# sandialabs/tenzing

Hardware: AMD Instinct MI355X
Metric: best-schedule iter time (ms) + MCTS search wall-clock, 3D halo-exchange 8 ranks (lower is better)
Workload: dtype fp64

## Files before the change

tenzing_amd/csrc/bind/module.cpp:

```cpp
#include <pybind11/functional.h>
#include <pybind11/numpy.h>
#include <pybind11/pybind11.h>
#include <pybind11/stl.h>

#include "core/benchmark.hpp"
#include "core/health.hpp"
#include "core/solve.hpp"
#include "hip/comm_ops.hpp"
#include "hip/hip_runtime.hpp"
#include "hip/rccl_comm.hpp"
#include "hip/rocsparse_spmv.hpp"
#include "kernels/kernels.hpp"
#include "workloads/workloads.hpp"

#include <hip/hip_runtime_api.h>

#include <csignal>
#include <cstdlib>
#include <execinfo.h>
#include <sstream>
#include <unistd.h>
#include <vector>

namespace py = pybind11;
// ... 1127 lines not shown
     "symmetric, strictly diagonally dominant band matrix (mirrored random_band_matrix off-diagonals, "
     "a_ii = 1 + sum |a_ij|) as (rowPtr, colInd, val)");
  py::class_<CgArgs>(m, "CgArgs")
      .def(py::init<>())
      .def_readwrite("m", &CgArgs::m)
      .def_readwrite("bw", &CgArgs::bw)
      .def_readwrite("nnz", &CgArgs::nnz)
      .def_readonly("nnz_actual", &CgArgs::nnz_actual)
      .def_readwrite("seed", &CgArgs::seed)
      .def_readwrite("matrix", &CgArgs::matrix)
      .def_readwrite("device", &CgArgs::device)
      .def_readwrite("form", &CgArgs::form)
      .def_readwrite("lanes", &CgArgs::lanes)
      .def_readwrite("rhs", &CgArgs::rhs)
      .def_readwrite("nrhs", &CgArgs::nrhs)
      .def_readwrite("rhs_first", &CgArgs::rhs_first)
      .def_readwrite("prefix", &CgArgs::prefix)
      .def_readwrite("rank", &CgArgs::rank)
      .def_readwrite("size", &CgArgs::size)
      .def("json", [](const CgArgs &a) { return a.json().dump(); });
  {
    auto f32 = [](const std::vector<float> &v) { return py::array_t<float>(py::ssize_t(v.size()), v.data()); };
    py::class_<ConjugateGradient, std::shared_ptr<ConjugateGradient>>(m, "ConjugateGradient")
        .def(py::init([](const CgArgs &a) { return std::make_shared<ConjugateGradient>(a); }), py::arg("args"))
        .def_property_readonly("args", &ConjugateGradient::args)
        .def("rows", &ConjugateGradient::rows)
        .def("matrix", [](const ConjugateGradient &c) {
          const CsrHost &a = c.matrix();
          return py::make_tuple(a.rowPtr, a.colInd, a.val);
        }, "the system matrix as (rowPtr, colInd, val)")
        .def("setup", &ConjugateGradient::setup, py::call_guard<py::gil_scoped_release>())
        .def("ready", &ConjugateGradient::ready)
        .def("add_to_graph", &ConjugateGradient::add_to_graph)
        .def("reset", &ConjugateGradient::reset, py::call_guard<py::gil_scoped_release>(),
             "x = 0, r = p = b, rr = b . b (synchronous)")
        .def("x", [f32](const ConjugateGradient &c, int col) { return f32(c.x(col)); }, py::arg("col") = 0,
             "column col (0 .. nrhs - 1) of x, de-interleaved; likewise r, p, b, rr, check and residual")
        .def("r", [f32](const ConjugateGradient &c, int col) { return f32(c.r(col)); }, py::arg("col") = 0)
        .def("p", [f32](const ConjugateGradient &c, int col) { return f32(c.p(col)); }, py::arg("col") = 0)
        .def("b", [f32](const ConjugateGradient &c, int col) { return f32(c.b(col)); }, py::arg("col") = 0)
        .def("rr", &ConjugateGradient::rr, py::arg("col") = 0,
             "r . r of the current residual (f64, the kernels' summation order)")
        .def("check", &ConjugateGradient::check, py::arg("k"), py::arg("col") = 0,
             py::call_guard<py::gil_scoped_release>(),
             "max |x - x_ref| / max |x_ref| against k host iterations in f64")
        .def("residual", &ConjugateGradient::residual, py::arg("col") = 0,
             py::call_guard<py::gil_scoped_release>(),
             "the true residual ||b - A x|| / ||b|| of the current x, in f64 on the host");
  }
  m.def("read_matrix_market", [](const std::string &path) {
    CsrHost a = read_matrix_market(path);
    return py::make_tuple(a.rows, a.cols, a.rowPtr, a.colInd, a.val);
  }, py::arg("path"));
  m.def("write_matrix_market", [](int64_t rows, int64_t cols, std::vector<int32_t> rowPtr,
                                  std::vector<int32_t> colInd, std::vector<float> val,
                                  const std::string &path) {
    CsrHost a;
    a.rows = rows;
    a.cols = cols;
    a.rowPtr = std::move(rowPtr);
    a.colInd = std::move(colInd);
    a.val = std::move(val);
    TZ_CHECK(int64_t(a.rowPtr.size()) == rows + 1 && a.colInd.size() == a.val.size() &&
                 int64_t(a.colInd.size()) == int64_t(a.rowPtr.back()),
             "inconsistent CSR arrays");
    write_matrix_market(a, path);
  }, py::arg("rows"), py::arg("cols"), py::arg("row_ptr"), py::arg("col_ind"), py::arg("val"), py::arg("path"));
  m.def("row_partition", &row_partition);

  auto k = m.def_submodule("kernels", "hand-written gfx950 kernels (raw device pointers)");
  k.def("box_copy", [](uintptr_t grid, py::dict d, bool unpack, uintptr_t s) {
    kern::box_copy(reinterpret_cast<double *>(grid), box_from_dict(d), unpack, P(s));
  }, py::arg("grid"), py::arg("box"), py::arg("unpack"), py::arg("stream") = 0);
  k.def("box_copy_many", [](uintptr_t grid, std::vector<py::dict> ds, bool unpack, uintptr_t s) {
    std::vector<kern::BoxDesc> bs;
    for (auto &d : ds) bs.push_back(box_from_dict(d));
    kern::box_copy_many(reinterpret_cast<double *>(grid), bs.data(), int(bs.size()), unpack, P(s));
  }, py::arg("grid"), py::arg("boxes"), py::arg("unpack"), py::arg("stream") = 0);
  k.def("csr_spmv", [](int n, uintptr_t rp, uintptr_t ci, uintptr_t v, uintptr_t x, uintptr_t y, int lanes, bool acc, uintptr_t s) {
    kern::csr_spmv(n, reinterpret_cast<const int32_t *>(rp), reinterpret_cast<const int32_t *>(ci),
                   reinterpret_cast<const float *>(v), reinterpret_cast<const float *>(x),
                   reinterpret_cast<float *>(y), lanes, acc, P(s));
  }, py::arg("n_rows"), py::arg("row_ptr"), py::arg("col_ind"), py::arg("val"), py::arg("x"), py::arg("y"),
     py::arg("lanes") = 0, py::arg("accumulate") = false, py::arg("stream") = 0);
  py::class_<RocsparseCsr, std::shared_ptr<RocsparseCsr>>(
      k, "RocsparseCsr", "rocSPARSE CSR SpMV (library comparison variant): y = A x on raw pointers")
      .def(py::init([](int64_t m, int64_t n, int64_t nnz, uintptr_t rp, uintptr_t ci, uintptr_t v,
                       uintptr_t x, uintptr_t y, const std::string &alg) {
             return std::make_shared<RocsparseCsr>(
                 m, n, nnz, reinterpret_cast<const int32_t *>(rp), reinterpret_cast<const int32_t *>(ci),
                 reinterpret_cast<const float *>(v), reinterpret_cast<const float *>(x),
                 reinterpret_cast<float *>(y), alg.c_str());
           }),
           py::arg("m"), py::arg("n"), py::arg("nnz"), py::arg("row_ptr"), py::arg("col_ind"),
           py::arg("val"), py::arg("x"), py::arg("y"), py::arg("alg") = "adaptive")
      .def("run", [](const RocsparseCsr &r, uintptr_t s, bool acc) { r.run(P(s), acc); },
           py::arg("stream") = 0, py::arg("accumulate") = false);
  k.def("stencil7", [](uintptr_t in, uintptr_t out, int64_t base, int row, int ny, int nz,
                       int nouter, int64_t sy, int64_t sz, int64_t so, int xs, double c0, double c1,
                       bool lds, uintptr_t s, int m0, int m1) {
    kern::StencilBox b;
    b.in = reinterpret_cast<const double *>(in);
    b.out = reinterpret_cast<double *>(out);
    b.base = base;
    b.row = row;
    b.ny = ny;
    b.nz = nz;
    b.nouter = nouter;
    b.sy = sy;
    b.sz = sz;
    b.so = so;
    b.xs = xs;
    b.c0 = c0;
    b.c1 = c1;
    b.m0 = m0;
    b.m1 = m1;
    kern::stencil7(b, lds, P(s));
  }, py::arg("in_"), py::arg("out"), py::arg("base"), py::arg("row"), py::arg("ny"), py::arg("nz"),
     py::arg("nouter"), py::arg("sy"), py::arg("sz"), py::arg("so"), py::arg("xs"),
     py::arg("c0") = 0.4, py::arg("c1") = 0.1, py::arg("lds") = true, py::arg("stream") = 0,
     py::arg("m0") = 0, py::arg("m1") = 0);
  k.def("stencil_thin", [](int row, int ny, int nz) {
    kern::StencilBox b;
    b.row = row;
    b.ny = ny;
    b.nz = nz;
    return kern::stencil_thin(b);
  }, py::arg("row"), py::arg("ny"), py::arg("nz"),
     "whether stencil7 sends a box of these extents to the one-thread-per-element kernel");
  k.def("stencil7_thin_many", [](uintptr_t in, uintptr_t out, std::vector<py::dict> ds, uintptr_t s) {
    std::vector<kern::StencilBox> bs;
    for (auto &d : ds) {
      kern::StencilBox b;
      b.in = reinterpret_cast<const double *>(in);
      b.out = reinterpret_cast<double *>(out);
      b.base = d["base"].cast<int64_t>();
      b.sy = d["sy"].cast<int64_t>();
      b.sz = d["sz"].cast<int64_t>();
      b.so = d["so"].cast<int64_t>();
      b.row = d["row"].cast<int>();
      b.ny = d["ny"].cast<int>();
      b.nz = d["nz"].cast<int>();
      b.nouter = d["nouter"].cast<int>();
      b.xs = d["xs"].cast<int>();
      if (d.contains("m0")) b.m0 = d["m0"].cast<int>();
      if (d.contains("m1")) b.m1 = d["m1"].cast<int>();
      if (d.contains("c0")) b.c0 = d["c0"].cast<double>();
      if (d.contains("c1")) b.c1 = d["c1"].cast<double>();
      bs.push_back(b);
    }
    kern::stencil7_thin_many(bs.data(), int(bs.size()), P(s));
  }, py::arg("in_"), py::arg("out"), py::arg("boxes"), py::arg("stream") = 0,
     "the one-thread-per-element kernel over a list of boxes (dicts of the StencilBox fields)");
  k.def("set_stencil_tuning", [](int ty, int zc, int pf, bool db) {
    TZ_CHECK(ty == 8 || ty == 16, "stencil ty must be 8 or 16");
    TZ_CHECK(zc == 16 || zc == 32 || zc == 64 || zc == 128, "stencil zc must be 16, 32, 64 or 128");
    TZ_CHECK(zc != 128 || pf == 1, "stencil zc 128 takes pf 1");
    TZ_CHECK(pf == 1 || pf == 2, "stencil pf must be 1 or 2");
    kern::stencil_tuning().ty = ty;
    kern::stencil_tuning().zc = zc;
    kern::stencil_tuning().pf = pf;
    kern::stencil_tuning().db = db;
  }, py::arg("ty") = 16, py::arg("zc") = 64, py::arg("pf") = 1, py::arg("db") = true);
  k.def("set_stencil_xcd_tiles", [](bool on) { kern::stencil_tuning().xcd_tiles = on; }, py::arg("on"),
        "stencil tiles in XCD-contiguous order (each XCD a contiguous range of tiles)");
  k.def("get_stencil_xcd_tiles", []() { return kern::stencil_tuning().xcd_tiles; });
  k.attr("CG_MAX_PARTIALS") = kern::kCgMaxPartials;
  k.attr("SPMV_ILP") = kern::kSpmvIlp;
  k.def("dot_partial_count", &kern::dot_partial_count, py::arg("n"));
  k.def("spmv_dot_partial_count", &kern::spmv_dot_partial_count, py::arg("n_rows"), py::arg("lanes"));
  k.def("dot_partials_f32", [](int64_t n, uintptr_t u, uintptr_t v, uintptr_t part, uintptr_t s) {
    kern::dot_partials_f32(n, reinterpret_cast<const float *>(u), reinterpret_cast<const float *>(v),
                           reinterpret_cast<double *>(part), P(s));
  }, py::arg("n"), py::arg("u"), py::arg("v"), py::arg("partials"), py::arg("stream") = 0);
  k.def("sum_partials_f64", [](uintptr_t part, int np, uintptr_t out, uintptr_t s) {
    kern::sum_partials_f64(reinterpret_cast<const double *>(part), np, reinterpret_cast<double *>(out), P(s));
  }, py::arg("partials"), py::arg("np"), py::arg("out"), py::arg("stream") = 0);
  k.def("cg_alpha", [](uintptr_t part, int np, uintptr_t rr, uintptr_t alpha, uintptr_t s) {
    kern::cg_alpha(reinterpret_cast<const double *>(part), np, reinterpret_cast<const double *>(rr),
                   reinterpret_cast<double *>(alpha), P(s));
  }, py::arg("partials_pq"), py::arg("np"), py::arg("rr"), py::arg("alpha"), py::arg("stream") = 0);
  k.def("cg_beta", [](uintptr_t part, int np, uintptr_t rr, uintptr_t beta, uintptr_t s) {
    kern::cg_beta(reinterpret_cast<const double *>(part), np, reinterpret_cast<double *>(rr),
                  reinterpret_cast<double *>(beta), P(s));
  }, py::arg("partials_rr"), py::arg("np"), py::arg("rr"), py::arg("beta"), py::arg("stream") = 0);
  k.def("axpy_dev_f32", [](int64_t n, uintptr_t sc, int sign, uintptr_t x, uintptr_t y, uintptr_t s) {
    kern::axpy_dev_f32(n, reinterpret_cast<const double *>(sc), sign, reinterpret_cast<const float *>(x),
                       reinterpret_cast<float *>(y), P(s));
  }, py::arg("n"), py::arg("scalar"), py::arg("sign"), py::arg("x"), py::arg("y"), py::arg("stream") = 0);
  k.def("xpay_dev_f32", [](int64_t n, uintptr_t sc, uintptr_t x, uintptr_t y, uintptr_t s) {
    kern::xpay_dev_f32(n, reinterpret_cast<const double *>(sc), reinterpret_cast<const float *>(x),
                       reinterpret_cast<float *>(y), P(s));
  }, py::arg("n"), py::arg("scalar"), py::arg("x"), py::arg("y"), py::arg("stream") = 0);
  k.def("csr_spmv_dot", [](int n, uintptr_t rp, uintptr_t ci, uintptr_t v, uintptr_t p, uintptr_t q, int lanes,
                           uintptr_t pq, uintptr_t prr, int npRr, uintptr_t rr, uintptr_t s) {
    kern::csr_spmv_dot(n, reinterpret_cast<const int32_t *>(rp), reinterpret_cast<const int32_t *>(ci),
                       reinterpret_cast<const float *>(v), reinterpret_cast<const float *>(p),
                       reinterpret_cast<float *>(q), lanes, reinterpret_cast<double *>(pq),
                       reinterpret_cast<const double *>(prr), npRr, reinterpret_cast<double *>(rr), P(s));
  }, py::arg("n_rows"), py::arg("row_ptr"), py::arg("col_ind"), py::arg("val"), py::arg("p"), py::arg("q"),
     py::arg("lanes"), py::arg("partials_pq"), py::arg("partials_rr") = 0, py::arg("np_rr") = 0,
     py::arg("rr") = 0, py::arg("stream") = 0);
  k.def("cg_fused_x", [](int64_t n, uintptr_t pq, int np, uintptr_t rr, uintptr_t p, uintptr_t x, uintptr_t s) {
    kern::cg_fused_x(n, reinterpret_cast<const double *>(pq), np, reinterpret_cast<const double *>(rr),
                     reinterpret_cast<const float *>(p), reinterpret_cast<float *>(x), P(s));
  }, py::arg("n"), py::arg("partials_pq"), py::arg("np"), py::arg("rr"), py::arg("p"), py::arg("x"),
     py::arg("stream") = 0);
  k.def("cg_fused_r", [](int64_t n, uintptr_t pq, int np, uintptr_t rr, uintptr_t q, uintptr_t r, uintptr_t prr,
                         uintptr_t s) {
    kern::cg_fused_r(n, reinterpret_cast<const double *>(pq), np, reinterpret_cast<const double *>(rr),
                     reinterpret_cast<const float *>(q), reinterpret_cast<float *>(r),
                     reinterpret_cast<double *>(prr), P(s));
  }, py::arg("n"), py::arg("partials_pq"), py::arg("np"), py::arg("rr"), py::arg("q"), py::arg("r"),
     py::arg("partials_rr"), py::arg("stream") = 0);
  k.def("cg_fused_p", [](int64_t n, uintptr_t prr, int np, uintptr_t rr, uintptr_t r, uintptr_t p, uintptr_t s) {
    kern::cg_fused_p(n, reinterpret_cast<const double *>(prr), np, reinterpret_cast<const double *>(rr),
                     reinterpret_cast<const float *>(r), reinterpret_cast<float *>(p), P(s));
  }, py::arg("n"), py::arg("partials_rr"), py::arg("np"), py::arg("rr"), py::arg("r"), py::arg("p"),
     py::arg("stream") = 0);
  k.def("csr_spmv_dot2", [](int n, uintptr_t rp, uintptr_t ci, uintptr_t v, uintptr_t r, uintptr_t w, int lanes,
                            uintptr_t pg, uintptr_t pd, uintptr_t gOut, uintptr_t aOut, uintptr_t gPrev,
                            uintptr_t aPrev, uintptr_t s) {
    kern::csr_spmv_dot2(n, reinterpret_cast<const int32_t *>(rp), reinterpret_cast<const int32_t *>(ci),
                        reinterpret_cast<const float *>(v), reinterpret_cast<const float *>(r),
                        reinterpret_cast<float *>(w), lanes, reinterpret_cast<double *>(pg),
                        reinterpret_cast<double *>(pd), reinterpret_cast<const double *>(gOut),
                        reinterpret_cast<const double *>(aOut), reinterpret_cast<double *>(gPrev),
                        reinterpret_cast<double *>(aPrev), P(s));
  }, py::arg("n_rows"), py::arg("row_ptr"), py::arg("col_ind"), py::arg("val"), py::arg("r"), py::arg("w"),
     py::arg("lanes"), py::arg("partials_gamma"), py::arg("partials_delta"), py::arg("gamma_out") = 0,
     py::arg("alpha_out") = 0, py::arg("gamma_prev") = 0, py::arg("alpha_prev") = 0, py::arg("stream") = 0);
  k.def("cg_sr_update", [](int64_t n, uintptr_t pg, uintptr_t pd, int np, uintptr_t gPrev, uintptr_t aPrev,
                           uintptr_t w, uintptr_t r, uintptr_t p, uintptr_t sv, uintptr_t x, uintptr_t gOut,
                           uintptr_t aOut, uintptr_t bOut, uintptr_t s) {
    kern::cg_sr_update(n, reinterpret_cast<const double *>(pg), reinterpret_cast<const double *>(pd), np,
                       reinterpret_cast<const double *>(gPrev), reinterpret_cast<const double *>(aPrev),
                       reinterpret_cast<const float *>(w), reinterpret_cast<float *>(r),
                       reinterpret_cast<float *>(p), reinterpret_cast<float *>(sv), reinterpret_cast<float *>(x),
                       reinterpret_cast<double *>(gOut), reinterpret_cast<double *>(aOut),
                       reinterpret_cast<double *>(bOut), P(s));
  }, py::arg("n"), py::arg("partials_gamma"), py::arg("partials_delta"), py::arg("np"), py::arg("gamma_prev"),
     py::arg("alpha_prev"), py::arg("w"), py::arg("r"), py::arg("p"), py::arg("s"), py::arg("x"),
     py::arg("gamma_out"), py::arg("alpha_out"), py::arg("beta_out"), py::arg("stream") = 0);
  k.def("csr_spmm_dot2", [](int n, uintptr_t rp, uintptr_t ci, uintptr_t v, uintptr_t r, uintptr_t w, int nrhs,
                            int lanes, uintptr_t pg, uintptr_t pd, uintptr_t gOut, uintptr_t aOut,
                            uintptr_t gPrev, uintptr_t aPrev, uintptr_t s) {
    kern::csr_spmm_dot2(n, reinterpret_cast<const int32_t *>(rp), reinterpret_cast<const int32_t *>(ci),
                        reinterpret_cast<const float *>(v), reinterpret_cast<const float *>(r),
                        reinterpret_cast<float *>(w), nrhs, lanes, reinterpret_cast<double *>(pg),
                        reinterpret_cast<double *>(pd), reinterpret_cast<const double *>(gOut),
                        reinterpret_cast<const double *>(aOut), reinterpret_cast<double *>(gPrev),
                        reinterpret_cast<double *>(aPrev), P(s));
  }, py::arg("n_rows"), py::arg("row_ptr"), py::arg("col_ind"), py::arg("val"), py::arg("r"), py::arg("w"),
     py::arg("k"), py::arg("lanes"), py::arg("partials_gamma"), py::arg("partials_delta"),
     py::arg("gamma_out") = 0, py::arg("alpha_out") = 0, py::arg("gamma_prev") = 0, py::arg("alpha_prev") = 0,
     py::arg("stream") = 0);
  k.def("cg_sr_update_batch", [](int64_t n, int nrhs, uintptr_t pg, uintptr_t pd, int np, uintptr_t gPrev,
                                 uintptr_t aPrev, uintptr_t w, uintptr_t r, uintptr_t p, uintptr_t sv, uintptr_t x,
                                 uintptr_t gOut, uintptr_t aOut, uintptr_t bOut, uintptr_t s) {
    kern::cg_sr_update_batch(n, nrhs, reinterpret_cast<const double *>(pg), reinterpret_cast<const double *>(pd),
                             np, reinterpret_cast<const double *>(gPrev), reinterpret_cast<const double *>(aPrev),
                             reinterpret_cast<const float *>(w), reinterpret_cast<float *>(r),
                             reinterpret_cast<float *>(p), reinterpret_cast<float *>(sv),
                             reinterpret_cast<float *>(x), reinterpret_cast<double *>(gOut),
                             reinterpret_cast<double *>(aOut), reinterpret_cast<double *>(bOut), P(s));
  }, py::arg("n"), py::arg("k"), py::arg("partials_gamma"), py::arg("partials_delta"), py::arg("np"),
     py::arg("gamma_prev"), py::arg("alpha_prev"), py::arg("w"), py::arg("r"), py::arg("p"), py::arg("s"),
     py::arg("x"), py::arg("gamma_out"), py::arg("alpha_out"), py::arg("beta_out"), py::arg("stream") = 0);
  k.def("gather_f32", [](int n, uintptr_t src, uintptr_t idx, uintptr_t dst, uintptr_t s) {
    kern::gather_f32(n, reinterpret_cast<const float *>(src), reinterpret_cast<const int32_t *>(idx),
                     reinterpret_cast<float *>(dst), P(s));
  }, py::arg("n"), py::arg("src"), py::arg("idx"), py::arg("dst"), py::arg("stream") = 0);
  k.def("vector_add_f32", [](int n, uintptr_t a, uintptr_t b, uintptr_t y, uintptr_t s) {
    kern::vector_add_f32(n, reinterpret_cast<const float *>(a), reinterpret_cast<const float *>(b),
                         reinterpret_cast<float *>(y), P(s));
  }, py::arg("n"), py::arg("a"), py::arg("b"), py::arg("y"), py::arg("stream") = 0);
  k.def("axpy_f64", [](int64_t n, double alpha, uintptr_t x, uintptr_t y, uintptr_t s) {
    kern::axpy_f64(n, alpha, reinterpret_cast<const double *>(x), reinterpret_cast<double *>(y), P(s));
  }, py::arg("n"), py::arg("alpha"), py::arg("x"), py::arg("y"), py::arg("stream") = 0);
  k.def("iota_f64", [](int64_t n, double base, double scale, uintptr_t a, uintptr_t s) {
    kern::iota_f64(n, base, scale, reinterpret_cast<double *>(a), P(s));
  }, py::arg("n"), py::arg("base"), py::arg("scale"), py::arg("a"), py::arg("stream") = 0);
  k.def("empty", [](uintptr_t s) { kern::empty(P(s)); }, py::arg("stream") = 0);
  auto moves_from = [](const std::vector<py::dict> &ds) {
    std::vector<kern::MoveDesc> ms;
    for (auto &d : ds) {
      kern::MoveDesc m;
      m.src = reinterpret_cast<const double *>(d["src"].cast<uintptr_t>());
      m.dst = reinterpret_cast<double *>(d["dst"].cast<uintptr_t>());
      m.src_off = d["src_off"].cast<int64_t>();
      m.dst_off = d["dst_off"].cast<int64_t>();
      m.s1 = d.contains("s1") ? d["s1"].cast<int64_t>() : 0;
      m.s2 = d.contains("s2") ? d["s2"].cast<int64_t>() : 0;
      m.s3 = d.contains("s3") ? d["s3"].cast<int64_t>() : 0;
      m.len = d["len"].cast<int32_t>();
      m.n1 = d.contains("n1") ? d["n1"].cast<int32_t>() : 1;
      m.n2 = d.contains("n2") ? d["n2"].cast<int32_t>() : 1;
      m.n3 = d.contains("n3") ? d["n3"].cast<int32_t>() : 1;
      m.pair = d.contains("pair") && d["pair"].cast<bool>();
      ms.push_back(m);
    }
    return ms;
  };
  k.def("box_move_spmv", [moves_from](std::vector<py::dict> ds, int n, uintptr_t rp, uintptr_t ci, uintptr_t v,
                                      uintptr_t x, uintptr_t y, int lanes, bool acc, uintptr_t s) {
    const std::vector<kern::MoveDesc> ms = moves_from(ds);
    kern::SpmvJob j;
    j.nRows = n;
    j.rowPtr = reinterpret_cast<const int32_t *>(rp);
    j.colInd = reinterpret_cast<const int32_t *>(ci);
    j.val = reinterpret_cast<const float *>(v);
    j.x = reinterpret_cast<const float *>(x);
    j.y = reinterpret_cast<float *>(y);
    j.lanes = lanes;
    j.accumulate = acc;
    kern::box_move_spmv(ms.data(), int(ms.size()), j, P(s));
// ... 175 lines not shown
```

tenzing_amd/csrc/kernels/kernels.hpp:

```cpp
#pragma once

#include <cstdint>
#include <vector>
#include <string>

namespace tz {
namespace kern {

struct BoxDesc {
  double *buf = nullptr;
  int64_t grid_off = 0;
  int64_t s1 = 0, s2 = 0, s3 = 0;
  int32_t len = 0, n1 = 0, n2 = 0, n3 = 0;
  int32_t lead = 0, trail = 0;
};

constexpr int kMaxBoxes = 32;

struct BoxTuning {
  int unroll = 3;
  bool nt_pack = true;
  bool nt_unpack = true;
  int max_blocks = 4096;
  int put_max_blocks = 64;
  bool nt_move = false;
  bool nt_move_store = true;
  int move_unroll = 1;
  int move_items = 2;
  int xcd_remap = 0;
  bool peel_moves = true;
  bool widen_unpack = true;
};
BoxTuning &box_tuning();
void set_xcd_remap(int mode);

struct MoveDesc {
  const double *src = nullptr;
  double *dst = nullptr;
  int64_t src_off = 0, dst_off = 0;
  int64_t s1 = 0, s2 = 0, s3 = 0;
  int32_t len = 0, n1 = 0, n2 = 0, n3 = 0;
  bool pair = false;
};
constexpr int kMaxPairLen = 8;
void box_move_many(const MoveDesc *d, int n, void *stream);

struct LineBox {
  double *base = nullptr;
  int64_t off = 0, s1 = 0, s2 = 0, s3 = 0;
  int32_t lines = 0, n1 = 0, n2 = 0, n3 = 0;
  int mode = 0;
  double *dst_base = nullptr;
  int64_t dst_off = 0;
};
constexpr int kLineRoofVariants = 4;
void line_roof(const LineBox *boxes, int n, void *stream, int variant = 0);
std::vector<LineBox> line_boxes(const MoveDesc *moves, int n, bool copies = true);
std::vector<std::string> move_kinds(const MoveDesc *moves, int n);

struct MoveSignal {
  unsigned int *done = nullptr;
  unsigned long long *flag[kMaxBoxes] = {};
  unsigned long long *count = nullptr;
  uint64_t store_mask = 0;
  int max_blocks = 0;
};
void box_move_many_signal(const MoveDesc *d, int n, const MoveSignal &sig, void *stream);
void box_pack_many_signal(double *grid, const BoxDesc *d, int n, const MoveSignal &sig,
                          void *stream);

void ipc_wait(const unsigned long long *arrive, unsigned long long *expected, const int *slots,
              int n, int *err, double timeout_s, void *stream, int lag = 0,
              unsigned long long *const *signal = nullptr);
void ipc_signal(unsigned long long *const *signal, int n, void *stream,
                unsigned long long *count = nullptr);

void box_copy(double *grid, const BoxDesc &d, bool unpack, void *stream);
void box_copy_many(double *grid, const BoxDesc *d, int n, bool unpack, void *stream);

void copy_bytes(void *dst, const void *src, size_t bytes, void *stream);
struct CopyDesc {
  void *dst = nullptr;
  const void *src = nullptr;
  size_t bytes = 0;
};
void copy_many(const CopyDesc *d, int n, void *stream);

constexpr int kSpmvIlp = 1000;
void csr_spmv(int nRows, const int32_t *rowPtr, const int32_t *colInd, const float *val,
              const float *x, float *y, int lanesPerRow, bool accumulate, void *stream);
struct SpmvJob {
  int nRows = 0;
  const int32_t *rowPtr = nullptr, *colInd = nullptr;
  const float *val = nullptr, *x = nullptr;
  float *y = nullptr;
  int lanes = kSpmvIlp + 4;
  bool accumulate = false;
};
void box_move_spmv(const MoveDesc *moves, int n, const SpmvJob &job, void *stream);
void gather_f32(int n, const float *src, const int32_t *idx, float *dst, void *stream);
struct PutSeg {
  float *dst = nullptr;
  int32_t off = 0, n = 0;
  unsigned long long *flag = nullptr;
};
constexpr int kMaxPutPeers = 64;
void gather_put_signal(const float *src, const int32_t *idx, const PutSeg *segs, int nseg,
                       unsigned int *done, void *stream);
void vector_add_f32(int n, const float *a, const float *b, float *y, void *stream);
constexpr int kCgMaxPartials = 256;
int dot_partial_count(int64_t n);
int spmv_dot_partial_count(int nRows, int lanes);
void dot_partials_f32(int64_t n, const float *u, const float *v, double *partials, void *stream);
void sum_partials_f64(const double *partials, int np, double *out, void *stream);
void cg_alpha(const double *partials_pq, int np, const double *rr, double *alpha, void *stream);
void cg_beta(const double *partials_rr, int np, double *rr, double *beta, void *stream);
void axpy_dev_f32(int64_t n, const double *s, int sign, const float *x, float *y, void *stream);
void xpay_dev_f32(int64_t n, const double *s, const float *x, float *y, void *stream);
void csr_spmv_dot(int nRows, const int32_t *rowPtr, const int32_t *colInd, const float *val, const float *p,
                  float *q, int lanes, double *partials_pq, const double *partials_rr, int np_rr, double *rr,
                  void *stream);
void cg_fused_x(int64_t n, const double *partials_pq, int np, const double *rr, const float *p, float *x,
                void *stream);
void cg_fused_r(int64_t n, const double *partials_pq, int np, const double *rr, const float *q, float *r,
                double *partials_rr, void *stream);
void cg_fused_p(int64_t n, const double *partials_rr, int np, const double *rr, const float *r, float *p,
                void *stream);
void csr_spmv_dot2(int nRows, const int32_t *rowPtr, const int32_t *colInd, const float *val, const float *r,
                   float *w, int lanes, double *partials_gamma, double *partials_delta, const double *gamma_out,
                   const double *alpha_out, double *gamma_prev, double *alpha_prev, void *stream);
void cg_sr_update(int64_t n, const double *partials_gamma, const double *partials_delta, int np,
                  const double *gamma_prev, const double *alpha_prev, const float *w, float *r, float *p, float *s,
                  float *x, double *gamma_out, double *alpha_out, double *beta_out, void *stream);
void csr_spmm_dot2(int nRows, const int32_t *rowPtr, const int32_t *colInd, const float *val, const float *R,
                   float *Wout, int k, int lanes, double *partials_gamma, double *partials_delta,
                   const double *gamma_out, const double *alpha_out, double *gamma_prev, double *alpha_prev,
                   void *stream);
void cg_sr_update_batch(int64_t n, int k, const double *partials_gamma, const double *partials_delta, int np,
                        const double *gamma_prev, const double *alpha_prev, const float *W, float *R, float *P,
                        float *S, float *X, double *gamma_out, double *alpha_out, double *beta_out, void *stream);

void axpy_f64(int64_t n, double alpha, const double *x, double *y, void *stream);
void iota_f64(int64_t n, double base, double scale, double *a, void *stream);
void empty(void *stream);
void busy_wait(int64_t ticks, int blocks, void *stream);

const int *abort_flag();
void set_abort(bool on);
bool abort_set();

struct StencilBox {
  const double *in = nullptr;
  double *out = nullptr;
  int64_t base = 0, sy = 0, sz = 0, so = 0;
  int32_t row = 0, ny = 0, nz = 0, nouter = 1, xs = 1;
  int32_t m0 = 0, m1 = 0;
  double c0 = 0.4, c1 = 0.1;
};
struct StencilTuning {
  int ty = 16;
  int zc = 64;
  int pf = 1;
  bool db = true;
  bool xcd_tiles = true;
};
StencilTuning &stencil_tuning();
void stencil7(const StencilBox &b, bool lds, void *stream);
bool stencil_thin(const StencilBox &b);
void stencil7_thin_many(const StencilBox *b, int n, void *stream);

struct HaloGeom {
  int32_t order = 0;
  int64_t xoff = 0, sy = 0, sz = 0, sq = 0;
  int32_t nx = 0, ny = 0, nz = 0, nq = 0, g = 0;
  int32_t cx = 0, cy = 0, cz = 0, px = 1, py = 1, pz = 1;
  int32_t neighbors = 6;
  int32_t gen = 0;
};
void halo_init(double *grid, const HaloGeom &g, void *stream);
void halo_check(const double *grid, const HaloGeom &g, unsigned long long *count, void *stream);
void stencil_check(const double *out, const HaloGeom &g, unsigned long long *count, void *stream);

}
}
```

tenzing_amd/csrc/kernels/stencil_kernels.hip:

```cpp
#include <hip/hip_runtime.h>

#include "kernels.hpp"
#include "launch.hpp"

#include <algorithm>
#include <cstdint>
#include <stdexcept>
#include <string>

namespace tz {
namespace kern {

namespace {

constexpr int TX = 64, XS_MAX = 4;

__device__ __forceinline__ double ldnt(const double *p) { return __builtin_nontemporal_load(p); }

template <int VX> struct VT;
template <> struct VT<1> {
  using T = double;
  __device__ static T zero() { return 0.0; }
  __device__ static double get(const T &v, int) { return v; }
};
template <> struct VT<2> {
  using T = dbl2_t;
  __device__ static T zero() { return T{0.0, 0.0}; }
  __device__ static double get(const T &v, int k) { return k ? v.y : v.x; }
};

struct TileGrid {
  uint32_t gx, gy, gz, per;
};

template <bool LDS, int VX, int TY, int ZC, int PF, bool DB>
__global__ __launch_bounds__(TX *TY) void stencil7_k(StencilBox b, TileGrid tg) {
  uint32_t bx = blockIdx.x, by = blockIdx.y, bz = blockIdx.z;
  if (tg.per) {
    const uint32_t l = (blockIdx.x % 8u) * tg.per + blockIdx.x / 8u;
    if (l >= tg.gx * tg.gy * tg.gz) return;
    bx = l % tg.gx;
    by = (l / tg.gx) % tg.gy;
    bz = l / (tg.gx * tg.gy);
  }
  using V = VT<VX>;
  using T = typename V::T;
  constexpr int W = TX * VX;
  constexpr int LW = W + 2 * XS_MAX;
  __shared__ double tiles[LDS && DB ? 2 : 1][TY + 2][LW];
  const int tx = threadIdx.x % TX, ty = threadIdx.x / TX;
  const int r = int(bx) * W + tx * VX;
  const int y = int(by) * TY + ty;
  const int zChunks = (b.nz + ZC - 1) / ZC;
  const int outer = int(bz) / zChunks;
  const int z0 = (int(bz) % zChunks) * ZC;
  const int z1 = min(z0 + ZC, b.nz);
  const int rlo = b.m0, rhi = b.row - b.m1;
  const bool mine = r + VX > rlo && r < rhi && y < b.ny;
  const int llo = rlo - b.xs, lhi = rhi + b.xs;
  const bool live = LDS ? (r + VX > llo && r < lhi && y <= b.ny) : mine;
  const int64_t e0 = b.base + int64_t(outer) * b.so + int64_t(y) * b.sy + r;
  const double *in = b.in;
  auto load = [&](int64_t e) { return *reinterpret_cast<const T *>(in + e); };

  constexpr int NAPRON = 2 * LW + 2 * TY * XS_MAX;
  constexpr int NT = TX * TY;
  int alr[2], alc[2], agr[2], agy[2];
  bool aok[2];
#pragma unroll
  for (int a = 0; a < 2; ++a) {
    const int k = threadIdx.x + a * NT;
    int lr = 0, lc = 0;
    if (k < 2 * LW) {
      lr = k < LW ? 0 : TY + 1;
      lc = k % LW;
    } else if (k < NAPRON) {
      const int j = k - 2 * LW;
      lr = 1 + j / (2 * XS_MAX);
      const int c = j % (2 * XS_MAX);
      lc = c < XS_MAX ? c : W + c;
    }
    alr[a] = lr;
    alc[a] = lc;
    agr[a] = int(bx) * W + lc - XS_MAX;
    agy[a] = int(by) * TY + lr - 1;
    aok[a] = LDS && k < NAPRON && agr[a] >= llo && agr[a] < lhi && agy[a] >= -1 && agy[a] <= b.ny;
  }
  const int64_t pbase = b.base + int64_t(outer) * b.so;
  auto apron = [&](int a, int z) {
    return aok[a] ? in[pbase + int64_t(z) * b.sz + int64_t(agy[a]) * b.sy + agr[a]] : 0.0;
  };

  auto loadnt = [&](int zz) {
    return live && zz <= b.nz
               ? __builtin_nontemporal_load(reinterpret_cast<const T *>(in + e0 + int64_t(zz) * b.sz))
               : V::zero();
  };
  T prev = mine ? load(e0 + int64_t(z0 - 1) * b.sz) : V::zero();
  T cur = live ? load(e0 + int64_t(z0) * b.sz) : V::zero();
  T next = live ? load(e0 + int64_t(z0 + 1) * b.sz) : V::zero();
  T ahead[PF];
#pragma unroll
  for (int p = 0; p + 1 < PF; ++p) ahead[p] = loadnt(z0 + 2 + p);
  double ap0 = apron(0, z0), ap1 = apron(1, z0);
  for (int z = z0; z < z1; ++z) {
    const int64_t e = e0 + int64_t(z) * b.sz;
    ahead[PF - 1] = loadnt(z + 1 + PF);
    auto &tile = tiles[LDS && DB ? (z - z0) & 1 : 0];
    double xm[VX], xp[VX], ym[VX], yp[VX];
    if (LDS) {
#pragma unroll
      for (int k = 0; k < VX; ++k) tile[ty + 1][XS_MAX + tx * VX + k] = V::get(cur, k);
      if (aok[0]) tile[alr[0]][alc[0]] = ap0;
      if (aok[1]) tile[alr[1]][alc[1]] = ap1;
      if (z + 1 < z1) {
        ap0 = apron(0, z + 1);
        ap1 = apron(1, z + 1);
      }
      __syncthreads();
#pragma unroll
      for (int k = 0; k < VX; ++k) {
        const int c = XS_MAX + tx * VX + k;
        xm[k] = tile[ty + 1][c - b.xs];
        xp[k] = tile[ty + 1][c + b.xs];
        ym[k] = tile[ty][c];
        yp[k] = tile[ty + 2][c];
      }
    } else {
#pragma unroll
      for (int k = 0; k < VX; ++k) {
        xm[k] = mine ? in[e + k - b.xs] : 0.0;
        xp[k] = mine ? in[e + k + b.xs] : 0.0;
        ym[k] = mine ? in[e + k - b.sy] : 0.0;
        yp[k] = mine ? in[e + k + b.sy] : 0.0;
      }
    }
    if (mine) {
      T o;
      if constexpr (VX == 1) {
        o = b.c0 * cur + b.c1 * (xm[0] + xp[0] + ym[0] + yp[0] + prev + next);
        __builtin_nontemporal_store(o, b.out + e);
      } else {
        o.x = b.c0 * cur.x + b.c1 * (xm[0] + xp[0] + ym[0] + yp[0] + prev.x + next.x);
        o.y = b.c0 * cur.y + b.c1 * (xm[1] + xp[1] + ym[1] + yp[1] + prev.y + next.y);
        if (r >= rlo && r + 1 < rhi) {
          __builtin_nontemporal_store(o, reinterpret_cast<T *>(b.out + e));
        } else {
          if (r >= rlo) b.out[e] = o.x;
          if (r + 1 >= rlo && r + 1 < rhi) b.out[e + 1] = o.y;
        }
      }
    }
    if (LDS && !DB) __syncthreads();
    prev = cur;
    cur = next;
    next = ahead[0];
#pragma unroll
    for (int p = 0; p + 1 < PF; ++p) ahead[p] = ahead[p + 1];
  }
}

constexpr int kMaxFlat = 8;
struct FlatBatch {
  StencilBox b[kMaxFlat];
  uint32_t block_start[kMaxFlat + 1];
  int32_t n;
};

__device__ __forceinline__ void flat_one(const StencilBox &b, int64_t it) {
  const int64_t i = it % b.row;
  if (i < b.m0 || i >= b.row - b.m1) return;
  int64_t r = it / b.row;
  const int64_t y = r % b.ny;
  r /= b.ny;
  const int64_t z = r % b.nz;
  const int64_t o = r / b.nz;
  const int64_t e = b.base + o * b.so + z * b.sz + y * b.sy + i;
  const double *in = b.in;
  b.out[e] = b.c0 * in[e] + b.c1 * (in[e - b.xs] + in[e + b.xs] + in[e - b.sy] + in[e + b.sy] +
                                    in[e - b.sz] + in[e + b.sz]);
}

__global__ __launch_bounds__(kThreads) void stencil7_flat_k(FlatBatch fb) {
  const BlockSlot s = find_block(fb.block_start, fb.n, blockIdx.x);
  const StencilBox &b = fb.b[s.entry];
  const int64_t total = int64_t(b.row) * b.ny * b.nz * b.nouter;
  const int64_t nth = int64_t(s.nb) * kThreads;
  int64_t it = int64_t(s.blk) * kThreads + threadIdx.x;
  for (; it + 3 * nth < total; it += 4 * nth) {
#pragma unroll
    for (int u = 0; u < 4; ++u) flat_one(b, it + u * nth);
  }
  for (; it < total; it += nth) flat_one(b, it);
}

}

bool stencil_thin(const StencilBox &b) { return b.nz < 4 || b.ny < 4 || b.row < 32; }

void stencil7_thin_many(const StencilBox *boxes, int n, void *stream) {
  hipStream_t s = static_cast<hipStream_t>(stream);
  for (int k = 0; k < n;) {
    FlatBatch fb{};
    for (; k < n && fb.n < kMaxFlat; ++k) {
      const StencilBox &b = boxes[k];
      const int64_t items = int64_t(b.row) * b.ny * b.nz * b.nouter;
      if (items <= 0) continue;
      if (!b.in || !b.out) throw std::runtime_error("stencil7: null grid");
      const uint32_t blocks = uint32_t(std::min<int64_t>((items + 1023) / 1024, 8192));
      fb.b[append_blocks(fb.block_start, fb.n, blocks)] = b;
    }
    if (fb.n == 0) continue;
    hipLaunchKernelGGL(stencil7_flat_k, dim3(fb.block_start[fb.n]), dim3(kThreads), 0, s, fb);
    TZ_HIP_LAUNCH_CHECK();
  }
}

StencilTuning &stencil_tuning() {
  static StencilTuning t;
  return t;
}

namespace {
template <bool LDS, int VX, int TY, int ZC, int PF, bool DB>
void launch_stencil_db(const StencilBox &b, hipStream_t s) {
  const int W = TX * VX;
  const int zChunks = (b.nz + ZC - 1) / ZC;
  TileGrid tg{unsigned((b.row + W - 1) / W), unsigned((b.ny + TY - 1) / TY), unsigned(zChunks * b.nouter), 0};
  dim3 g(tg.gx, tg.gy, tg.gz);
  if (stencil_tuning().xcd_tiles) {
    const uint64_t total = uint64_t(tg.gx) * tg.gy * tg.gz;
    if (total >= (uint64_t(1) << 31)) throw std::runtime_error("stencil7: too many tiles");
    tg.per = unsigned((total + 7) / 8);
    g = dim3(tg.per * 8);
  }
  hipLaunchKernelGGL((stencil7_k<LDS, VX, TY, ZC, PF, DB>), g, dim3(TX * TY), 0, s, b, tg);
}

template <bool LDS, int VX, int TY, int ZC, int PF>
void launch_stencil(const StencilBox &b, hipStream_t s) {
  if (stencil_tuning().db) launch_stencil_db<LDS, VX, TY, ZC, PF, true>(b, s);
  else launch_stencil_db<LDS, VX, TY, ZC, PF, false>(b, s);
}

template <bool LDS, int VX, int TY>
void launch_zc(const StencilBox &b, hipStream_t s) {
  const StencilTuning &t = stencil_tuning();
  if (t.zc == 64) {
    if (t.pf >= 2) launch_stencil<LDS, VX, TY, 64, 2>(b, s);
    else launch_stencil<LDS, VX, TY, 64, 1>(b, s);
  } else if (t.zc == 128) {
    launch_stencil<LDS, VX, TY, 128, 1>(b, s);
  } else if (t.zc == 16) {
    if (t.pf >= 2) launch_stencil<LDS, VX, TY, 16, 2>(b, s);
    else launch_stencil<LDS, VX, TY, 16, 1>(b, s);
  } else {
    if (t.pf >= 2) launch_stencil<LDS, VX, TY, 32, 2>(b, s);
    else launch_stencil<LDS, VX, TY, 32, 1>(b, s);
  }
}

template <bool LDS, int VX>
void launch_ty(const StencilBox &b, hipStream_t s) {
  const StencilTuning &t = stencil_tuning();
  if (t.ty == 16) launch_zc<LDS, VX, 16>(b, s);
  else launch_zc<LDS, VX, 8>(b, s);
}
}

void stencil7(const StencilBox &b, bool lds, void *stream) {
  if (b.row <= 0 || b.ny <= 0 || b.nz <= 0 || b.nouter <= 0) return;
  if (!b.in || !b.out) throw std::runtime_error("stencil7: null grid");
  if (b.xs < 1 || b.xs > XS_MAX) throw std::runtime_error("stencil7: x neighbour distance must be 1..4");
  const bool v2 = b.row % 2 == 0 && b.base % 2 == 0 && b.sy % 2 == 0 && b.sz % 2 == 0 &&
                  b.so % 2 == 0 && reinterpret_cast<uintptr_t>(b.in) % 16 == 0 &&
                  reinterpret_cast<uintptr_t>(b.out) % 16 == 0;
  hipStream_t s = static_cast<hipStream_t>(stream);
  if (stencil_thin(b)) {
    stencil7_thin_many(&b, 1, stream);
    return;
  }
  if (lds && v2) launch_ty<true, 2>(b, s);
  else if (lds) launch_ty<true, 1>(b, s);
  else if (v2) launch_ty<false, 2>(b, s);
  else launch_ty<false, 1>(b, s);
  TZ_HIP_LAUNCH_CHECK();
}

}
}
```

Before: 0.04415.

## Register-block z-march stencil over kx by ky outputs per thread

Each thread of the LDS z-march stencil now computes a KX by KY block of outputs (default 2x2), giving larger tiles with a proportionally smaller apron. In-thread y neighbours come from registers rather than LDS, and the z chunk size becomes a runtime parameter instead of a template argument. The aim is to raise per-thread work and data reuse and to shrink the share of halo loads. The cost is more registers per thread, larger LDS tiles and fewer, bigger blocks, which on small halo-exchange grids could reduce parallelism or occupancy.

```diff
diff --git a/tenzing_amd/csrc/bind/module.cpp b/tenzing_amd/csrc/bind/module.cpp
--- a/tenzing_amd/csrc/bind/module.cpp
+++ b/tenzing_amd/csrc/bind/module.cpp
@@ -1303,16 +1303,37 @@
     kern::stencil7_thin_many(bs.data(), int(bs.size()), P(s));
   }, py::arg("in_"), py::arg("out"), py::arg("boxes"), py::arg("stream") = 0,
      "the one-thread-per-element kernel over a list of boxes (dicts of the StencilBox fields)");
-  k.def("set_stencil_tuning", [](int ty, int zc, int pf, bool db) {
+  const kern::StencilTuning st0;
+  k.def("set_stencil_tuning", [](int ty, int zc, int pf, bool db, int kx, int ky) {
     TZ_CHECK(ty == 8 || ty == 16, "stencil ty must be 8 or 16");
     TZ_CHECK(zc == 16 || zc == 32 || zc == 64 || zc == 128, "stencil zc must be 16, 32, 64 or 128");
     TZ_CHECK(zc != 128 || pf == 1, "stencil zc 128 takes pf 1");
     TZ_CHECK(pf == 1 || pf == 2, "stencil pf must be 1 or 2");
-    kern::stencil_tuning().ty = ty;
-    kern::stencil_tuning().zc = zc;
-    kern::stencil_tuning().pf = pf;
-    kern::stencil_tuning().db = db;
-  }, py::arg("ty") = 16, py::arg("zc") = 64, py::arg("pf") = 1, py::arg("db") = true);
+    kern::StencilTuning t = kern::stencil_tuning();
+    t.ty = ty;
+    t.zc = zc;
+    t.pf = pf;
+    t.db = db;
+    t.kx = kx;
+    t.ky = ky;
+    kern::stencil_tuning_check(t);
+    kern::stencil_tuning() = t;
+  }, py::arg("ty") = st0.ty, py::arg("zc") = st0.zc, py::arg("pf") = st0.pf, py::arg("db") = st0.db,
+     py::arg("kx") = st0.kx, py::arg("ky") = st0.ky,
+     "launch shape of the z-march stencil: 64 x ty threads, tiles of 128 * kx elements by ty * ky rows");
+  k.def("get_stencil_tuning", []() {
+    const kern::StencilTuning &t = kern::stencil_tuning();
+    py::dict d;
+    d["ty"] = t.ty;
+    d["zc"] = t.zc;
+    d["pf"] = t.pf;
+    d["db"] = t.db;
+    d["xcd_tiles"] = t.xcd_tiles;
+    d["kx"] = t.kx;
+    d["ky"] = t.ky;
+    d["lds_bytes"] = kern::stencil_lds_bytes(t);
+    return d;
+  }, "the whole stencil tuning as a dict, with the LDS bytes of its tile");
   k.def("set_stencil_xcd_tiles", [](bool on) { kern::stencil_tuning().xcd_tiles = on; }, py::arg("on"),
         "stencil tiles in XCD-contiguous order (each XCD a contiguous range of tiles)");
   k.def("get_stencil_xcd_tiles", []() { return kern::stencil_tuning().xcd_tiles; });
diff --git a/tenzing_amd/csrc/kernels/kernels.hpp b/tenzing_amd/csrc/kernels/kernels.hpp
--- a/tenzing_amd/csrc/kernels/kernels.hpp
+++ b/tenzing_amd/csrc/kernels/kernels.hpp
@@ -163,8 +163,12 @@
   int pf = 1;
   bool db = true;
   bool xcd_tiles = true;
+  int kx = 2;
+  int ky = 2;
 };
 StencilTuning &stencil_tuning();
+size_t stencil_lds_bytes(const StencilTuning &t);
+void stencil_tuning_check(const StencilTuning &t);
 void stencil7(const StencilBox &b, bool lds, void *stream);
 bool stencil_thin(const StencilBox &b);
 void stencil7_thin_many(const StencilBox *b, int n, void *stream);
diff --git a/tenzing_amd/csrc/kernels/stencil_kernels.hip b/tenzing_amd/csrc/kernels/stencil_kernels.hip
--- a/tenzing_amd/csrc/kernels/stencil_kernels.hip
+++ b/tenzing_amd/csrc/kernels/stencil_kernels.hip
@@ -14,8 +14,13 @@
 namespace {
 
 constexpr int TX = 64, XS_MAX = 4;
-
-__device__ __forceinline__ double ldnt(const double *p) { return __builtin_nontemporal_load(p); }
+constexpr size_t kLdsMax = 160 * 1024;
+constexpr int kMaxTileWork = 64;
+
+__device__ __forceinline__ double point7(double c0, double c1, double cur, double xm, double xp, double ym,
+                                         double yp, double prev, double next) {
+  return c0 * cur + c1 * (xm + xp + ym + yp + prev + next);
+}
 
 template <int VX> struct VT;
 template <> struct VT<1> {
@@ -31,9 +36,14 @@
 
 struct TileGrid {
   uint32_t gx, gy, gz, per;
+  int32_t zc;
 };
 
-template <bool LDS, int VX, int TY, int ZC, int PF, bool DB>
+constexpr size_t tile_bytes(int vx, int ty, int kx, int ky, bool db) {
+  return size_t(db ? 2 : 1) * size_t(ty * ky + 2) * size_t(TX * vx * kx + 2 * XS_MAX) * sizeof(double);
+}
+
+template <bool LDS, int VX, int TY, int KX, int KY, int PF, bool DB>
 __global__ __launch_bounds__(TX *TY) void stencil7_k(StencilBox b, TileGrid tg) {
   uint32_t bx = blockIdx.x, by = blockIdx.y, bz = blockIdx.z;
   if (tg.per) {
@@ -45,118 +55,168 @@
   }
   using V = VT<VX>;
   using T = typename V::T;
-  constexpr int W = TX * VX;
+  constexpr int SEG = TX * VX;
+  constexpr int W = SEG * KX;
+  constexpr int H = TY * KY;
   constexpr int LW = W + 2 * XS_MAX;
-  __shared__ double tiles[LDS && DB ? 2 : 1][TY + 2][LW];
+  static_assert(!LDS || tile_bytes(VX, TY, KX, KY, DB) <= kLdsMax, "stencil7: tile exceeds the LDS");
+  __shared__ double tiles[LDS && DB ? 2 : 1][H + 2][LW];
   const int tx = threadIdx.x % TX, ty = threadIdx.x / TX;
-  const int r = int(bx) * W + tx * VX;
-  const int y = int(by) * TY + ty;
-  const int zChunks = (b.nz + ZC - 1) / ZC;
+  const int r0 = int(bx) * W + tx * VX;
+  const int y0 = int(by) * H + ty * KY;
+  const int zChunks = (b.nz + tg.zc - 1) / tg.zc;
   const int outer = int(bz) / zChunks;
-  const int z0 = (int(bz) % zChunks) * ZC;
-  const int z1 = min(z0 + ZC, b.nz);
+  const int z0 = (int(bz) % zChunks) * tg.zc;
+  const int z1 = min(z0 + tg.zc, b.nz);
   const int rlo = b.m0, rhi = b.row - b.m1;
-  const bool mine = r + VX > rlo && r < rhi && y < b.ny;
   const int llo = rlo - b.xs, lhi = rhi + b.xs;
-  const bool live = LDS ? (r + VX > llo && r < lhi && y <= b.ny) : mine;
-  const int64_t e0 = b.base + int64_t(outer) * b.so + int64_t(y) * b.sy + r;
+  bool cmine[KX], clive[KX], ymine[KY], ylive[KY];
+#pragma unroll
+  for (int j = 0; j < KX; ++j) {
+    const int r = r0 + j * SEG;
+    cmine[j] = r + VX > rlo && r < rhi;
+    clive[j] = LDS ? (r + VX > llo && r < lhi) : cmine[j];
+  }
+#pragma unroll
+  for (int i = 0; i < KY; ++i) {
+    ymine[i] = y0 + i < b.ny;
+    ylive[i] = LDS ? y0 + i <= b.ny : ymine[i];
+  }
+  const int64_t pbase = b.base + int64_t(outer) * b.so;
+  const int64_t e00 = pbase + int64_t(y0) * b.sy + r0;
   const double *in = b.in;
+  auto off = [&](int i, int j) { return e00 + int64_t(i) * b.sy + j * SEG; };
   auto load = [&](int64_t e) { return *reinterpret_cast<const T *>(in + e); };
 
-  constexpr int NAPRON = 2 * LW + 2 * TY * XS_MAX;
+  constexpr int NAPRON = 2 * W + 2 * H * XS_MAX;
   constexpr int NT = TX * TY;
-  int alr[2], alc[2], agr[2], agy[2];
-  bool aok[2];
-#pragma unroll
-  for (int a = 0; a < 2; ++a) {
+  constexpr int NA = (NAPRON + NT - 1) / NT;
+  int alds[NA];
+  int64_t aglb[NA];
+  bool aok[NA];
+#pragma unroll
+  for (int a = 0; a < NA; ++a) {
     const int k = threadIdx.x + a * NT;
     int lr = 0, lc = 0;
-    if (k < 2 * LW) {
-      lr = k < LW ? 0 : TY + 1;
-      lc = k % LW;
-    } else if (k < NAPRON) {
-      const int j = k - 2 * LW;
+    bool ok = LDS && k < NAPRON;
+    if (k < 2 * W) {
+      lr = k < W ? 0 : H + 1;
+      lc = XS_MAX + k % W;
+    } else {
+      const int j = k - 2 * W;
       lr = 1 + j / (2 * XS_MAX);
       const int c = j % (2 * XS_MAX);
       lc = c < XS_MAX ? c : W + c;
     }
-    alr[a] = lr;
-    alc[a] = lc;
-    agr[a] = int(bx) * W + lc - XS_MAX;
-    agy[a] = int(by) * TY + lr - 1;
-    aok[a] = LDS && k < NAPRON && agr[a] >= llo && agr[a] < lhi && agy[a] >= -1 && agy[a] <= b.ny;
-  }
-  const int64_t pbase = b.base + int64_t(outer) * b.so;
-  auto apron = [&](int a, int z) {
-    return aok[a] ? in[pbase + int64_t(z) * b.sz + int64_t(agy[a]) * b.sy + agr[a]] : 0.0;
-  };
-
-  auto loadnt = [&](int zz) {
-    return live && zz <= b.nz
-               ? __builtin_nontemporal_load(reinterpret_cast<const T *>(in + e0 + int64_t(zz) * b.sz))
+    const int gr = int(bx) * W + lc - XS_MAX, gy = int(by) * H + lr - 1;
+    if (k < 2 * W) ok = ok && gr >= rlo && gr < rhi && gy >= -1 && gy <= b.ny;
+    else ok = ok && gr >= llo && gr < lhi && gy < b.ny && (lc < XS_MAX ? lc >= XS_MAX - b.xs : lc < W + XS_MAX + b.xs);
+    alds[a] = lr * LW + lc;
+    aglb[a] = pbase + int64_t(gy) * b.sy + gr;
+    aok[a] = ok;
+  }
+  auto apron = [&](int a, int z) { return aok[a] ? in[aglb[a] + int64_t(z) * b.sz] : 0.0; };
+
+  auto loadnt = [&](int i, int j, int zz) {
+    return clive[j] && ylive[i] && zz <= b.nz
+               ? __builtin_nontemporal_load(reinterpret_cast<const T *>(in + off(i, j) + int64_t(zz) * b.sz))
                : V::zero();
   };
-  T prev = mine ? load(e0 + int64_t(z0 - 1) * b.sz) : V::zero();
-  T cur = live ? load(e0 + int64_t(z0) * b.sz) : V::zero();
-  T next = live ? load(e0 + int64_t(z0 + 1) * b.sz) : V::zero();
-  T ahead[PF];
-#pragma unroll
-  for (int p = 0; p + 1 < PF; ++p) ahead[p] = loadnt(z0 + 2 + p);
-  double ap0 = apron(0, z0), ap1 = apron(1, z0);
+  T prev[KY][KX], cur[KY][KX], next[KY][KX], ahead[PF][KY][KX];
+#pragma unroll
+  for (int i = 0; i < KY; ++i) {
+#pragma unroll
+    for (int j = 0; j < KX; ++j) {
+      const bool mine = cmine[j] && ymine[i], live = clive[j] && ylive[i];
+      prev[i][j] = mine ? load(off(i, j) + int64_t(z0 - 1) * b.sz) : V::zero();
+      cur[i][j] = live ? load(off(i, j) + int64_t(z0) * b.sz) : V::zero();
+      next[i][j] = live ? load(off(i, j) + int64_t(z0 + 1) * b.sz) : V::zero();
+#pragma unroll
+      for (int p = 0; p + 1 < PF; ++p) ahead[p][i][j] = loadnt(i, j, z0 + 2 + p);
+    }
+  }
+  double ap[NA];
+#pragma unroll
+  for (int a = 0; a < NA; ++a) ap[a] = apron(a, z0);
   for (int z = z0; z < z1; ++z) {
-    const int64_t e = e0 + int64_t(z) * b.sz;
-    ahead[PF - 1] = loadnt(z + 1 + PF);
+#pragma unroll
+    for (int i = 0; i < KY; ++i) {
+#pragma unroll
+      for (int j = 0; j < KX; ++j) ahead[PF - 1][i][j] = loadnt(i, j, z + 1 + PF);
+    }
     auto &tile = tiles[LDS && DB ? (z - z0) & 1 : 0];
-    double xm[VX], xp[VX], ym[VX], yp[VX];
     if (LDS) {
 #pragma unroll
-      for (int k = 0; k < VX; ++k) tile[ty + 1][XS_MAX + tx * VX + k] = V::get(cur, k);
-      if (aok[0]) tile[alr[0]][alc[0]] = ap0;
-      if (aok[1]) tile[alr[1]][alc[1]] = ap1;
+      for (int i = 0; i < KY; ++i) {
+#pragma unroll
+        for (int j = 0; j < KX; ++j) {
+#pragma unroll
+          for (int k = 0; k < VX; ++k)
+            tile[ty * KY + i + 1][XS_MAX + j * SEG + tx * VX + k] = V::get(cur[i][j], k);
+        }
+      }
+#pragma unroll
+      for (int a = 0; a < NA; ++a) {
+        if (aok[a]) (&tile[0][0])[alds[a]] = ap[a];
+      }
       if (z + 1 < z1) {
-        ap0 = apron(0, z + 1);
-        ap1 = apron(1, z + 1);
+#pragma unroll
+        for (int a = 0; a < NA; ++a) ap[a] = apron(a, z + 1);
       }
       __syncthreads();
-#pragma unroll
-      for (int k = 0; k < VX; ++k) {
-        const int c = XS_MAX + tx * VX + k;
-        xm[k] = tile[ty + 1][c - b.xs];
-        xp[k] = tile[ty + 1][c + b.xs];
-        ym[k] = tile[ty][c];
-        yp[k] = tile[ty + 2][c];
-      }
-    } else {
-#pragma unroll
-      for (int k = 0; k < VX; ++k) {
-        xm[k] = mine ? in[e + k - b.xs] : 0.0;
-        xp[k] = mine ? in[e + k + b.xs] : 0.0;
-        ym[k] = mine ? in[e + k - b.sy] : 0.0;
-        yp[k] = mine ? in[e + k + b.sy] : 0.0;
-      }
-    }
-    if (mine) {
-      T o;
-      if constexpr (VX == 1) {
-        o = b.c0 * cur + b.c1 * (xm[0] + xp[0] + ym[0] + yp[0] + prev + next);
-        __builtin_nontemporal_store(o, b.out + e);
-      } else {
-        o.x = b.c0 * cur.x + b.c1 * (xm[0] + xp[0] + ym[0] + yp[0] + prev.x + next.x);
-        o.y = b.c0 * cur.y + b.c1 * (xm[1] + xp[1] + ym[1] + yp[1] + prev.y + next.y);
-        if (r >= rlo && r + 1 < rhi) {
-          __builtin_nontemporal_store(o, reinterpret_cast<T *>(b.out + e));
-        } else {
-          if (r >= rlo) b.out[e] = o.x;
-          if (r + 1 >= rlo && r + 1 < rhi) b.out[e + 1] = o.y;
+    }
+#pragma unroll
+    for (int i = 0; i < KY; ++i) {
+#pragma unroll
+      for (int j = 0; j < KX; ++j) {
+        const bool mine = cmine[j] && ymine[i];
+        const int r = r0 + j * SEG;
+        const int64_t e = off(i, j) + int64_t(z) * b.sz;
+        double o[VX];
+#pragma unroll
+        for (int k = 0; k < VX; ++k) {
+          double xm, xp, ym, yp;
+          if (LDS) {
+            const int lr = ty * KY + i + 1, c = XS_MAX + j * SEG + tx * VX + k;
+            xm = tile[lr][c - b.xs];
+            xp = tile[lr][c + b.xs];
+            ym = i > 0 ? V::get(cur[i > 0 ? i - 1 : 0][j], k) : tile[lr - 1][c];
+            yp = i + 1 < KY ? V::get(cur[i + 1 < KY ? i + 1 : 0][j], k) : tile[lr + 1][c];
+          } else {
+            xm = mine ? in[e + k - b.xs] : 0.0;
+            xp = mine ? in[e + k + b.xs] : 0.0;
+            ym = mine ? in[e + k - b.sy] : 0.0;
+            yp = mine ? in[e + k + b.sy] : 0.0;
+          }
+          o[k] = point7(b.c0, b.c1, V::get(cur[i][j], k), xm, xp, ym, yp, V::get(prev[i][j], k),
+                        V::get(next[i][j], k));
         }
+        if (mine) {
+          if constexpr (VX == 1) {
+            __builtin_nontemporal_store(o[0], b.out + e);
+          } else {
+            if (r >= rlo && r + 1 < rhi) {
+              __builtin_nontemporal_store(T{o[0], o[1]}, reinterpret_cast<T *>(b.out + e));
+            } else {
+              if (r >= rlo) b.out[e] = o[0];
+              if (r + 1 >= rlo && r + 1 < rhi) b.out[e + 1] = o[1];
+            }
+          }
+        }
       }
     }
     if (LDS && !DB) __syncthreads();
-    prev = cur;
-    cur = next;
-    next = ahead[0];
-#pragma unroll
-    for (int p = 0; p + 1 < PF; ++p) ahead[p] = ahead[p + 1];
+#pragma unroll
+    for (int i = 0; i < KY; ++i) {
+#pragma unroll
+      for (int j = 0; j < KX; ++j) {
+        prev[i][j] = cur[i][j];
+        cur[i][j] = next[i][j];
+        next[i][j] = ahead[0][i][j];
+#pragma unroll
+        for (int p = 0; p + 1 < PF; ++p) ahead[p][i][j] = ahead[p + 1][i][j];
+      }
+    }
   }
 }
 
@@ -221,50 +281,85 @@
   return t;
 }
 
+size_t stencil_lds_bytes(const StencilTuning &t) { return tile_bytes(2, t.ty, t.kx, t.ky, t.db); }
+
+void stencil_tuning_check(const StencilTuning &t) {
+  auto bad = [](const std::string &what) { throw std::invalid_argument("stencil tuning: " + what); };
+  if (t.ty != 8 && t.ty != 16) bad("ty must be 8 or 16");
+  if (t.zc != 16 && t.zc != 32 && t.zc != 64 && t.zc != 128) bad("zc must be 16, 32, 64 or 128");
+  if (t.pf != 1 && t.pf != 2) bad("pf must be 1 or 2");
+  if (t.zc == 128 && t.pf != 1) bad("zc 128 takes pf 1");
+  if (t.kx != 1 && t.kx != 2 && t.kx != 4) bad("kx must be 1, 2 or 4");
+  if (t.ky != 1 && t.ky != 2 && t.ky != 4) bad("ky must be 1, 2 or 4");
+  const size_t need = stencil_lds_bytes(t);
+  if (need > kLdsMax)
+    bad("a " + std::to_string(2 * TX * t.kx) + " x " + std::to_string(t.ty * t.ky) + " tile" +
+        (t.db ? ", double-buffered," : "") + " needs " + std::to_string(need) + " bytes of LDS, a workgroup has " +
+        std::to_string(kLdsMax));
+  if (t.ty * t.kx * t.ky > kMaxTileWork)
+    bad("ty * kx * ky = " + std::to_string(t.ty * t.kx * t.ky) + " exceeds " + std::to_string(kMaxTileWork) +
+        ": the z queue of " + std::to_string(2 * t.kx * t.ky) + " elements per thread would spill");
+}
+
 namespace {
-template <bool LDS, int VX, int TY, int ZC, int PF, bool DB>
-void launch_stencil_db(const StencilBox &b, hipStream_t s) {
-  const int W = TX * VX;
-  const int zChunks = (b.nz + ZC - 1) / ZC;
-  TileGrid tg{unsigned((b.row + W - 1) / W), unsigned((b.ny + TY - 1) / TY), unsigned(zChunks * b.nouter), 0};
+template <bool LDS, int VX, int TY, int KX, int KY, int PF, bool DB>
+void launch_stencil(const StencilBox &b, hipStream_t s) {
+  const StencilTuning &t = stencil_tuning();
+  const int W = TX * VX * KX, H = TY * KY;
+  const int zChunks = (b.nz + t.zc - 1) / t.zc;
+  TileGrid tg{unsigned((b.row + W - 1) / W), unsigned((b.ny + H - 1) / H), unsigned(zChunks * b.nouter), 0, t.zc};
   dim3 g(tg.gx, tg.gy, tg.gz);
-  if (stencil_tuning().xcd_tiles) {
+  if (t.xcd_tiles) {
     const uint64_t total = uint64_t(tg.gx) * tg.gy * tg.gz;
     if (total >= (uint64_t(1) << 31)) throw std::runtime_error("stencil7: too many tiles");
     tg.per = unsigned((total + 7) / 8);
     g = dim3(tg.per * 8);
   }
-  hipLaunchKernelGGL((stencil7_k<LDS, VX, TY, ZC, PF, DB>), g, dim3(TX * TY), 0, s, b, tg);
-}
-
-template <bool LDS, int VX, int TY, int ZC, int PF>
-void launch_stencil(const StencilBox &b, hipStream_t s) {
-  if (stencil_tuning().db) launch_stencil_db<LDS, VX, TY, ZC, PF, true>(b, s);
-  else launch_stencil_db<LDS, VX, TY, ZC, PF, false>(b, s);
-}
-
-template <bool LDS, int VX, int TY>
-void launch_zc(const StencilBox &b, hipStream_t s) {
+  hipLaunchKernelGGL((stencil7_k<LDS, VX, TY, KX, KY, PF, DB>), g, dim3(TX * TY), 0, s, b, tg);
+}
+
+template <typename F> void dispatch_pf_db(F &&f) {
   const StencilTuning &t = stencil_tuning();
-  if (t.zc == 64) {
-    if (t.pf >= 2) launch_stencil<LDS, VX, TY, 64, 2>(b, s);
-    else launch_stencil<LDS, VX, TY, 64, 1>(b, s);
-  } else if (t.zc == 128) {
-    launch_stencil<LDS, VX, TY, 128, 1>(b, s);
-  } else if (t.zc == 16) {
-    if (t.pf >= 2) launch_stencil<LDS, VX, TY, 16, 2>(b, s);
-    else launch_stencil<LDS, VX, TY, 16, 1>(b, s);
-  } else {
-    if (t.pf >= 2) launch_stencil<LDS, VX, TY, 32, 2>(b, s);
-    else launch_stencil<LDS, VX, TY, 32, 1>(b, s);
-  }
-}
-
-template <bool LDS, int VX>
-void launch_ty(const StencilBox &b, hipStream_t s) {
+  dispatch_bools(t.pf >= 2 && t.zc != 128, t.db,
+                 [&](auto pf2, auto db) { f(Int<decltype(pf2)::value ? 2 : 1>{}, db); });
+}
+
+template <int TY, typename F> void dispatch_shape(F &&f) {
   const StencilTuning &t = stencil_tuning();
-  if (t.ty == 16) launch_zc<LDS, VX, 16>(b, s);
-  else launch_zc<LDS, VX, 8>(b, s);
+  auto go = [&](auto kx, auto ky) {
+    if constexpr (TY * decltype(kx)::value * decltype(ky)::value <= kMaxTileWork) f(kx, ky);
+    else throw std::runtime_error("stencil7: tile shape not offered (stencil_tuning_check)");
+  };
+  auto with_ky = [&](auto kx) {
+    if (t.ky == 1) go(kx, Int<1>{});
+    else if (t.ky == 2) go(kx, Int<2>{});
+    else if (t.ky == 4) go(kx, Int<4>{});
+    else throw std::runtime_error("stencil7: ky must be 1, 2 or 4");
+  };
+  if (t.kx == 1) with_ky(Int<1>{});
+  else if (t.kx == 2) with_ky(Int<2>{});
+  else if (t.kx == 4) with_ky(Int<4>{});
+  else throw std::runtime_error("stencil7: kx must be 1, 2 or 4");
+}
+
+template <int VX, int TY> void launch_lds(const StencilBox &b, hipStream_t s) {
+  dispatch_shape<TY>([&](auto kx, auto ky) {
+    dispatch_pf_db([&](auto pf, auto db) {
+      launch_stencil<true, VX, TY, decltype(kx)::value, decltype(ky)::value, decltype(pf)::value,
+                     decltype(db)::value>(b, s);
+    });
+  });
+}
+
+template <int VX, int TY> void launch_direct(const StencilBox &b, hipStream_t s) {
+  if (stencil_tuning().pf >= 2 && stencil_tuning().zc != 128) launch_stencil<false, VX, TY, 1, 1, 2, false>(b, s);
+  else launch_stencil<false, VX, TY, 1, 1, 1, false>(b, s);
+}
+
+template <int VX> void launch_ty(const StencilBox &b, bool lds, hipStream_t s) {
+  const bool ty16 = stencil_tuning().ty == 16;
+  if (lds) ty16 ? launch_lds<VX, 16>(b, s) : launch_lds<VX, 8>(b, s);
+  else ty16 ? launch_direct<VX, 16>(b, s) : launch_direct<VX, 8>(b, s);
 }
 }
 
@@ -280,10 +375,8 @@
     stencil7_thin_many(&b, 1, stream);
     return;
   }
-  if (lds && v2) launch_ty<true, 2>(b, s);
-  else if (lds) launch_ty<true, 1>(b, s);
-  else if (v2) launch_ty<false, 2>(b, s);
-  else launch_ty<false, 1>(b, s);
+  if (v2) launch_ty<2>(b, lds, s);
+  else launch_ty<1>(b, lds, s);
   TZ_HIP_LAUNCH_CHECK();
 }
 
```

Result: no change. 0.04410, median of 4 (-0.1%).
